# ccaven/tinyslam

Measured on AMD Instinct MI355X. Metric: ORB extract throughput, 1280x720 (frames/sec; Mkeypoints/sec alongside), higher is better.
Workload: dtype f32; 1 GPU; BASELINE.json configs[3]: batch of 256 independent 1280x720 RGBA frames per GPU, device-resident, full ORB (FAST-12 + orientation + blur + BRIEF-256); frames_per_gpu_per_batch=256, width=1280, height=720, hierarchy_depth=2, max_features=8192, content=default, mode=literal, input=rgba, pipeline=default, fp_contract=0, angle_bins=0, batches_in_flight=1, collate=none (1 GPU)

## Files before the change

tinyslam_amd/csrc/orb_api.hip:

```cpp
#include <hip/hip_runtime.h>
#include <chrono>
#include <cmath>

#include <cstdarg>
#include <cstdio>
#include <cstdlib>
#include <cstring>
#include <new>
#include <optional>
#include <string>
#include <algorithm>
#include <vector>

#include "../../include/tinyorb.h"
#include "orb_front_launch.h"
#include "orb_kernels_fused.h"
#include "orb_kernels_brief.h"
#include "orb_kernels_intended.h"
#include "orb_kernels_staged.h"
#include "orb_kernels_collate.h"
#include "orb_kernels_match.h"
#include "orb_kernels_verify.h"
#include "orb_kernels_epipolar.h"
#include "orb_kernels_guide.h"
// ... 84 lines not shown
    float* d_iseg_scores = nullptr;
    uint32_t* d_iseg_counts = nullptr;
    uint32_t* d_iseg_before = nullptr;
    unsigned long long* d_thr_key = nullptr;
    uint32_t ibrief_lds = 0;
    MatchRecord* d_matches = nullptr;
    uint8_t* d_desc8 = nullptr;
    int match_valu = -1;
    hipEvent_t match_done = nullptr;
    hipStream_t match_stream = nullptr;
    uint64_t batch_seq = 0;
    uint64_t match_seq = 0;
    uint32_t match_set = 0;
    uint32_t match_frames = 0;
    VerifierState verify, epi;
    uint4* d_gsrec = nullptr;
    uint4* d_gsdesc = nullptr;
    uint32_t* d_gcell = nullptr;
    MatchRecord* d_gmatch = nullptr;
    float* d_gmodel = nullptr;
    float* h_gmodel = nullptr;
    hipEvent_t guide_done = nullptr;
    hipStream_t guide_stream = nullptr;
    uint32_t guide_pairs = 0;
    int guide_cell = -1;
    uint64_t guide_seq = 0;
    uint32_t guide_set = 0;
    uint32_t* d_tkeys = nullptr;
    uint32_t* d_tprev = nullptr;
    uint32_t* d_tnext = nullptr;
    uint4* d_tptr = nullptr;
    uint4* d_track = nullptr;
    uint32_t* d_tlinks = nullptr;
    uint32_t* d_tshared = nullptr;
    uint32_t* d_tframe = nullptr;
    hipEvent_t track_done = nullptr;
    hipStream_t track_stream = nullptr;
    uint32_t track_frames = 0;
    int track_global_keys = -1;
    uint32_t* d_prov2_counts = nullptr;
    CornerData* d_prov2 = nullptr;
    float* d_prov2_scores = nullptr;

    uint8_t* d_input = nullptr;
    uint8_t* d_input_alt = nullptr;
    uint32_t in_last = 0;
    uint32_t in_pending = 0;
    uint32_t in_queue[2] = {0u, 0u};
    hipEvent_t in_uploaded[2] = {nullptr, nullptr};
    bool in_async[2] = {false, false};
    struct {
        bool single_memcpy = false, single_split = false, single_serial = false, single_sync = false, single_block = false;
        bool no_swizzle = false, quiet = false;
        int phase_mask = -1, brief_i_mask = -1, lds_pad = 0;
    } env;
    uint32_t* dv_count = nullptr;
    CornerData* dv_corners = nullptr;
    CornerDescriptor* dv_desc = nullptr;
    uint16_t* d_gray = nullptr;
    uint16_t* d_blur = nullptr;
    uint16_t* d_blur_rowc = nullptr;
    uint32_t blur_qa[kMaxLevels] = {0};
    uint32_t* d_counts = nullptr;
    CornerData* d_corners = nullptr;
    CornerDescriptor* d_desc = nullptr;
    uint32_t* out_counts[2] = {nullptr, nullptr};
    CornerData* out_corners[2] = {nullptr, nullptr};
    CornerDescriptor* out_desc[2] = {nullptr, nullptr};
    CornerData* d_seg = nullptr;
    uint32_t* d_seg_counts = nullptr;
    uint32_t* d_seg_before = nullptr;
    BandGeom bands{};
    RowsGeom rows{};
    BriefTGeom brieft{};
    bool use_brief_t = false;
    uint32_t band_rows_lvl[kMaxLevels] = {0};
    uint32_t ln_threads[kMaxLevels] = {0};
    uint32_t tile_w_lvl[kMaxLevels] = {0};
    uint32_t seg_classes = 1;
    uint32_t* d_pattern = nullptr;
    float* d_cos = nullptr;
    float* d_sin = nullptr;
    uint4* d_rot = nullptr;
    unsigned long long* d_stamps = nullptr;

    uint32_t* h_count = nullptr;
    uint32_t* d_single_done = nullptr;
    hipEvent_t single_done_ev = nullptr;
    uint32_t single_seq = 0;
    CornerData* h_corners = nullptr;
    CornerDescriptor* h_desc = nullptr;
    bool single_valid = false;

    uint32_t last_batch = 0;
    hipStream_t last_stream = nullptr;
    bool planes_valid = false;
    bool fused = false;
    uint32_t max_lds = 0;
    uint32_t n_cus = 256;

    bool profiling = false;
    std::vector<ProfSpan> pending;
    std::vector<hipEvent_t> event_pool;
    double prof_ms[ORB_KERNEL_COUNT] = {0};
    uint64_t prof_n[ORB_KERNEL_COUNT] = {0};

// ... 279 lines not shown
    g.rows_padded = rows;
    g.oob = p->oob;
    *out = g;
    if (getenv("TINYORB_BRIEF_ROWS")) return false;
    return rg.n_slots >= 1u && rg.n_slots * n_classes <= kBriefTMaxSlots && rows <= kBriefTMaxRows;
}

int launch_brief(OrbProgram* p, hipStream_t s, uint32_t n, const RowsGeom& rows_geom, const uint16_t* d_blur,
                 const uint16_t* d_blur_rowc, const uint32_t* seg_counts, uint32_t* seg_before, const CornerData* seg,
                 uint32_t* d_counts, CornerData* d_corners, CornerDescriptor* d_desc) {
    const uint32_t cap = p->cfg.max_features;
    const BriefTables tab{p->d_pattern, p->d_cos, p->d_sin, p->d_rot};
    const bool use_t = p->use_brief_t;
    {
        LaunchScope ls(p, s, KID_PREFIX);
        hipLaunchKernelGGL(k_slot_prefix, dim3(n), dim3(64), 0, s, seg_counts, seg_before, d_counts, rows_geom.n_slots,
                           rows_geom.seg_cap, use_t ? p->brieft.n_classes : 1u);
    }
    if (use_t) {
        const BriefTGeom& tg = p->brieft;
        const dim3 grid(n, (cap + (uint32_t)kBriefNfChunk - 1u) / (uint32_t)kBriefNfChunk);
        {
            LaunchScope ls(p, s, KID_BRIEF_T);
#define BRIEF_T_LAUNCH(ROT_)                                                                                                         \
    hipLaunchKernelGGL((k_brief_t<kBriefTWaves, ROT_>), dim3(n, (cap + kBriefTThreads - 1u) / kBriefTThreads), dim3(kBriefTThreads), \
                       brieft_lds_bytes(tg), s, d_blur_rowc, p->pyr, tg, seg_counts, seg_before, seg, d_corners, cap, d_desc, tab)
            switch (rot_form(p->opt.fp_contract)) {
                case 1: BRIEF_T_LAUNCH(1); break;
                case 2: BRIEF_T_LAUNCH(2); break;
                default: BRIEF_T_LAUNCH(0); break;
            }
#undef BRIEF_T_LAUNCH
        }
        LaunchScope ls(p, s, KID_BRIEF_NF);
        if (p->oob != kOobZero)
            hipLaunchKernelGGL(k_brief_nf<true>, grid, dim3(256), 0, s, d_blur, d_blur_rowc, p->pyr, tg, seg_counts, seg_before, d_corners,
                               cap, d_desc, tab);
        else
            hipLaunchKernelGGL(k_brief_nf<false>, grid, dim3(256), 0, s, d_blur, d_blur_rowc, p->pyr, tg, seg_counts, seg_before, d_corners,
                               cap, d_desc, tab);
    } else {
        LaunchScope ls(p, s, KID_BRIEF_ROWS);
        RowsGeom rg = rows_geom;
        rg.oob = p->oob;
        rg.fp = p->opt.fp_contract;
        rg.split = 1u;
        while (rg.split < 16u && rg.n_slots * n * rg.split < 2048u) rg.split *= 2u;
        hipLaunchKernelGGL(k_brief_rows, dim3(rg.n_slots * rg.split, n), dim3(256), 0, s, d_blur, d_blur_rowc, p->pyr, rg,
                           seg_counts, seg_before, seg, d_corners, cap, d_desc, tab);
    }
    return ORB_OK;
}

int run_fused_range(OrbProgram* p, const uint8_t* frames_all, uint32_t f0, uint32_t n, hipStream_t s, bool with_brief = true,
                    uint32_t first_level = 0) {
    const Pyramid& pyr = p->pyr;
    const uint32_t D = pyr.depth, cap = p->cfg.max_features;
    const uint8_t* frames = frames_all + (size_t)f0 * p->frame_bytes;
    uint16_t* const d_gray = p->d_gray + (size_t)f0 * pyr.stride;
    uint16_t* const d_blur = p->d_blur + (size_t)f0 * pyr.stride;
    uint16_t* const d_blur_rowc = p->d_blur_rowc + (size_t)f0 * pyr.row_stride;
    const size_t lists = (size_t)p->bands.n_slots * p->seg_classes;
    uint32_t* const d_seg_counts = p->d_seg_counts + (size_t)f0 * lists;
    uint32_t* const d_seg_before = p->d_seg_before + (size_t)f0 * lists;
    CornerData* const d_seg = p->d_seg + (size_t)f0 * lists * p->bands.seg_cap;
    uint32_t* const d_counts = p->d_counts + f0;
    CornerData* const d_corners = p->d_corners + (size_t)f0 * cap;
    CornerDescriptor* const d_desc = p->d_desc + (size_t)f0 * cap;
    uint32_t width = pyr.w[0], height = pyr.h[0];
    for (uint32_t lvl = 0; lvl < D; lvl++) {
        const uint32_t gw = ((width + 7u) / 8u) * 8u, gh = ((height + 7u) / 8u) * 8u;
        width /= 2u;
        height /= 2u;
        if (lvl < first_level) continue;
        if (lvl > 0 && !(pyr.w[lvl - 1] == 2u * pyr.w[lvl] && pyr.h[lvl - 1] == 2u * pyr.h[lvl])) {
            hipStream_t sm = s;
            LaunchScope ls(p, sm, KID_MIP);
            dim3 grid((pyr.w[lvl] + 63u) / 64u, (pyr.h[lvl] + 4u * kMipRows - 1u) / (4u * kMipRows), n);
            hipLaunchKernelGGL(k_mip, grid, dim3(64, 4), 0, sm, d_gray, pyr, lvl, (float)pyr.w[lvl - 1] / (float)pyr.w[lvl], (float)pyr.h[lvl - 1] / (float)pyr.h[lvl], p->wq);
        }
        FrontGeom g = front_geometry(pyr, lvl, gw ? gw : 8u, gh, n, p->band_rows_lvl[lvl], p->tile_w_lvl[lvl], p->ln_threads[lvl]);
        hipStream_t s_lvl = s;
        if (gw == 0) g.gh = 0;
        g.slot_base = p->bands.slot_base[lvl];
        g.n_slots = p->bands.n_slots;
        g.seg_cap = p->bands.seg_cap;
        g.n_classes = p->seg_classes;
        g.stamps = p->d_stamps;
        if (p->env.phase_mask >= 0) g.phase_mask = (uint32_t)p->env.phase_mask;
        if (p->env.no_swizzle) g.xcd_swizzle = 0u;
        g.oob = p->oob;
        g.wq = p->wq;
        g.fp = p->opt.fp_contract;
        g.store_grey = (lvl == 0 && D > 1 && !(pyr.w[0] == 2u * pyr.w[1] && pyr.h[0] == 2u * pyr.h[1])) ? 1u : 0u;
        if (g.n_bands * (g.tiled ? g.n_ct : 1u) != p->bands.slot_base[lvl + 1] - p->bands.slot_base[lvl])
            return fail(p, ORB_EINVAL, "internal: band count mismatch at level %u", lvl);
        if (!g.tiled && sizeof(BlurCol) * (size_t)g.n_var > 8u * (size_t)g.ts)
            return fail(p, ORB_EINVAL, "internal: blur column table of level %u does not fit", lvl);
        uint32_t lds = front_lds_bytes(g);
        lds += (uint32_t)p->env.lds_pad;
        if (lds > p->max_lds) return fail(p, ORB_EINVAL, "level %u needs %u bytes of LDS", lvl, lds);
        const dim3 grid(g.n_bands * (g.tiled ? g.n_ct : 1u) * n);
        FrontLaunch L{frames, p->frame_bytes, d_gray, d_blur, d_blur_rowc, pyr, g, p->threshold, d_seg_counts, d_seg, s_lvl, grid.x, lds,
                      p->band_rows_lvl[lvl], p->ln_threads[lvl], p->input_y8,
                      lvl == 0 && ((pyr.w[0] & 3u) || g.store_grey), p->oob != kOobZero, false};
        {
            LaunchScope ls(p, s_lvl, lvl == 0 ? KID_FUSED_L0 : KID_FUSED_LN);
            const hipError_t e = kFrontLaunch[front_form(p->opt.fp_contract, lvl == 0 && !p->input_y8)](L);
            if (e != hipSuccess) return fail(p, ORB_EHIP, "k_front (level %u) failed to launch: %s", lvl, hipGetErrorString(e));
        }
    }
    if (with_brief) launch_brief(p, s, n, p->rows, d_blur, d_blur_rowc, d_seg_counts, d_seg_before, d_seg, d_counts, d_corners, d_desc);
    HIP_TRY(p, hipGetLastError());
    return ORB_OK;
}

int run_fused(OrbProgram* p, const uint8_t* frames, uint32_t n, hipStream_t s) {
    if (int rc = run_fused_range(p, frames, 0, n, s)) return rc;
    p->planes_valid = true;
    return ORB_OK;
}

uint32_t itile_width(uint32_t w) {
    const uint32_t w8 = (w + 7u) & ~7u;
    return w8 < (uint32_t)kITileW ? w8 : (uint32_t)kITileW;
}

bool fused_i_eligible(const OrbProgram* p) {
    if (!p->intended || (p->opt.flags & ORB_FLAG_STAGED)) return false;
    const Pyramid& pyr = p->pyr;
    if ((uint64_t)pyr.w[0] * pyr.h[0] > (1ull << 26)) return false;
    if ((pyr.w[0] & 3u) != 0u || pyr.w[0] < 8u) return false;
    return true;
}

int run_fused_i(OrbProgram* p, const uint8_t* frames, uint32_t n, hipStream_t s) {
    const Pyramid& pyr = p->pyr;
    const uint32_t D = pyr.depth, cap = p->cfg.max_features;
    const IBriefGeom& bg = p->itiles;
    for (uint32_t lvl = 0; lvl < D; lvl++) {
        if (lvl > 0 && !(pyr.w[lvl - 1] == 2u * pyr.w[lvl] && pyr.h[lvl - 1] == 2u * pyr.h[lvl])) {
            LaunchScope ls(p, s, KID_MIP);
            dim3 grid((pyr.w[lvl] + 63u) / 64u, (pyr.h[lvl] + 4u * kMipRows - 1u) / (4u * kMipRows), n);
            hipLaunchKernelGGL(k_mip, grid, dim3(64, 4), 0, s, p->d_gray, pyr, lvl, (float)pyr.w[lvl - 1] / (float)pyr.w[lvl], (float)pyr.h[lvl - 1] / (float)pyr.h[lvl]);
        }
        IGeom g{};
        g.lvl = lvl;
        g.tw = bg.tw[lvl];
        g.n_ct = bg.n_ct[lvl];
        g.n_bands = (pyr.h[lvl] + kFrontRows - 1) / kFrontRows;
        g.ls = kIPad + g.tw + 16u;
        g.write_mip = (lvl + 1 < D && pyr.w[lvl] == 2u * pyr.w[lvl + 1] && pyr.h[lvl] == 2u * pyr.h[lvl + 1]) ? 1u : 0u;
        g.xcd_swizzle = (n % 8u == 0u) ? 1u : 0u;
        g.slot_base = bg.slot_base[lvl];
        g.n_slots = bg.n_slots;
        g.seg_cap = bg.seg_cap;
        g.arc = p->arc;
        g.nms = (p->opt.flags & ORB_FLAG_NMS) ? 1u : 0u;
// ... 175 lines not shown
    if (config->max_features == 0 || config->max_features > (1u << 24))
        return fail(nullptr, ORB_EINVAL, "max_features must be 1..=2^24");
    if (!(config->initial_threshold >= 0.f)) return fail(nullptr, ORB_EINVAL, "initial_threshold must be >= 0");
    if (options && options->fast_arc != 0 && (options->fast_arc < 9 || options->fast_arc > 16))
        return fail(nullptr, ORB_EINVAL, "fast_arc must be 0 (= 12) or 9..16");
    if (options && (options->flags & ORB_FLAG_INPUT_Y8) &&
        ((options->flags & (ORB_FLAG_INTENDED | ORB_FLAG_NMS)) || (options->fast_arc != 0 && options->fast_arc != 12)))
        return fail(nullptr, ORB_EINVAL, "ORB_FLAG_INPUT_Y8 is defined for the reference's detector only (no "
                                         "ORB_FLAG_INTENDED, ORB_FLAG_NMS or fast_arc other than 12)");
    if (options && (options->oob_policy > ORB_OOB_UMIN || options->sampler_weight_bits > 23u))
        return fail(nullptr, ORB_EINVAL, "oob_policy must be ORB_OOB_ZERO / _CLAMP / _UMIN and sampler_weight_bits 0..23");
    if (options && (options->oob_policy != ORB_OOB_ZERO || options->sampler_weight_bits != 0u) &&
        ((options->flags & (ORB_FLAG_INTENDED | ORB_FLAG_NMS)) || (options->fast_arc != 0 && options->fast_arc != 12)))
        return fail(nullptr, ORB_EINVAL, "oob_policy / sampler_weight_bits follow the reference's adapter: they are defined for the "
                                         "reference's detector only (no ORB_FLAG_INTENDED, ORB_FLAG_NMS or fast_arc other than 12)");
    if (options && options->fp_contract > (ORB_FP_CONTRACT_ALL | ORB_FP_LAST_TERM_FIRST))
        return fail(nullptr, ORB_EINVAL, "fp_contract is a mask of ORB_FP_CONTRACT_LUMINANCE / _BLUR / _ROTATION and ORB_FP_LAST_TERM_FIRST");
    if (options && options->fp_contract &&
        ((options->flags & (ORB_FLAG_INTENDED | ORB_FLAG_NMS | ORB_FLAG_INPUT_Y8)) || (options->fast_arc != 0 && options->fast_arc != 12)))
        return fail(nullptr, ORB_EINVAL, "fp_contract follows the reference's shader compiler: it is defined for the reference's detector on RGBA "
                                         "input only (no ORB_FLAG_INTENDED, ORB_FLAG_NMS, ORB_FLAG_INPUT_Y8 or fast_arc other than 12)");
    if (options && options->angle_bins && (!(options->flags & ORB_FLAG_INTENDED) || options->angle_bins < 8u || options->angle_bins > 6284u))
        return fail(nullptr, ORB_EINVAL, "angle_bins is an option of ORB_FLAG_INTENDED (IM-6b): 0, or 8..6284 bins of the full circle");
    if (options && (options->flags & ORB_FLAG_INTENDED) && (W > 16384u || H > 16384u))
        return fail(nullptr, ORB_EINVAL, "ORB_FLAG_INTENDED needs W, H <= 16384 (14-bit coordinates in the top-K key)");

    OrbProgram* p = new (std::nothrow) OrbProgram();
    if (!p) return fail(nullptr, ORB_EINVAL, "out of host memory");
    p->cfg = *config;
    if (options) p->opt = *options;
    p->device = p->opt.device;
    p->max_batch = p->opt.max_batch ? p->opt.max_batch : 1u;
    p->threshold = config->initial_threshold;
    p->intended = (p->opt.flags & ORB_FLAG_INTENDED) != 0u;
    p->input_y8 = (p->opt.flags & ORB_FLAG_INPUT_Y8) != 0u;
    p->arc = p->opt.fast_arc ? p->opt.fast_arc : (p->intended ? 9u : 12u);
    p->oob = p->opt.oob_policy;
    p->wq = p->opt.sampler_weight_bits ? (float)(1u << p->opt.sampler_weight_bits) : 0.0f;
    p->frame_bytes = (size_t)W * H * (p->input_y8 ? 1u : 4u);
    layout_pyramid(W, H, config->hierarchy_depth, &p->pyr);
    {
        auto on = [](const char* name) { const char* e = getenv(name); return e && *e && atoi(e) != 0; };
        auto num = [](const char* name, int dflt) { const char* e = getenv(name); return e && *e ? atoi(e) : dflt; };
        p->env.single_memcpy = on("TINYORB_SINGLE_MEMCPY");
        p->env.single_split = on("TINYORB_SINGLE_SPLIT");
        p->env.single_serial = on("TINYORB_SINGLE_SERIAL");
        p->env.single_sync = on("TINYORB_SINGLE_SYNC");
        {
            const char* w = getenv("TINYORB_SINGLE_WAIT");
            p->env.single_block = (w && !strcmp(w, "block")) || (p->opt.flags & ORB_FLAG_SINGLE_BLOCKING_WAIT) != 0u;
        }
        p->env.no_swizzle = on("TINYORB_NO_SWIZZLE");
        p->env.quiet = getenv("TINYORB_QUIET") != nullptr;
        p->env.phase_mask = num("TINYORB_PHASE_MASK", -1);
        p->env.brief_i_mask = num("TINYORB_BRIEF_I_MASK", -1);
        p->env.lds_pad = num("TINYORB_LDS_PAD", 0);
    }

    auto bail = [&](int code) {
        g_create_error = p->err;
        orb_program_destroy(p);
        return code;
    };
    int n_dev = 0;
    hipError_t e = hipGetDeviceCount(&n_dev);
    if (e != hipSuccess || n_dev <= 0) {
        fail(p, ORB_EHIP, "no HIP device available (%s)", e == hipSuccess ? "count is 0" : hipGetErrorString(e));
        return bail(ORB_EHIP);
    }
    if (p->device < 0 || p->device >= n_dev) {
        fail(p, ORB_EINVAL, "device %d out of range (0..%d)", p->device, n_dev - 1);
        return bail(ORB_EINVAL);
    }
#define CREATE_TRY(expr)                                                            \
    do {                                                                            \
        hipError_t e2_ = (expr);                                                    \
        if (e2_ != hipSuccess) {                                                    \
            fail(p, ORB_EHIP, "%s failed: %s", #expr, hipGetErrorString(e2_));      \
            return bail(ORB_EHIP);                                                  \
        }                                                                           \
    } while (0)
    CREATE_TRY(hipSetDevice(p->device));
    CREATE_TRY(hipStreamCreateWithFlags(&p->stream, hipStreamNonBlocking));
    {
        int lds_max = 0;
        CREATE_TRY(hipDeviceGetAttribute(&lds_max, hipDeviceAttributeMaxSharedMemoryPerBlock, p->device));
        p->max_lds = (uint32_t)lds_max;
        int cus = 0;
        CREATE_TRY(hipDeviceGetAttribute(&cus, hipDeviceAttributeMultiprocessorCount, p->device));
        p->n_cus = cus > 0 ? (uint32_t)cus : 256u;
        p->fused = fused_eligible(p);
        if (p->fused) {
            uint32_t need = 0;
            {
                uint32_t width = W, height = H;
                const char* force = getenv("TINYORB_BAND_ROWS");
                for (uint32_t lvl = 0; lvl < p->pyr.depth; lvl++) {
                    const uint32_t gw = ((width + 7u) / 8u) * 8u, gh = ((height + 7u) / 8u) * 8u, w = p->pyr.w[lvl];
                    width /= 2u;
                    height /= 2u;
                    uint32_t rows = 0, rows_lds = 0, fits = 0, fits_lds = 0, want = 0, want_lds = 0;
                    const uint32_t forced = force ? (uint32_t)atoi(force) : 0u;
                    auto pick = [&](uint32_t threads) {
                        rows = rows_lds = fits = fits_lds = want = want_lds = 0u;
                        for (int cand : kFrontBandHeights) {
                            if (std::max(w, gw) > (1u << front_x_bits(cand)) || std::max(w, gw) > (uint32_t)kFrontMaxWidthWide) continue;
// ... 28 lines not shown
                            tw = std::min(dom, (((dom + n_ct - 1u) / n_ct) + 7u) & ~7u);
                            t_rows = 0;
                            for (uint32_t cand : {16u, 8u}) {
                                const FrontGeom tg = front_geometry(p->pyr, lvl, gw, gh, 1, cand, tw);
                                const uint32_t lds = front_lds_bytes(tg);
                                const uint32_t items = lvl == 0 ? (tg.tw + 12u) / 4u : (tg.tw + 20u) / 8u;
                                if (!front_tile0_holds_blur(tg, w) || cand > (1u << (15u - tg.xb)) || lds > p->max_lds ||
                                    items > (lvl == 0 ? (uint32_t)kFrontThreadsL0 : (uint32_t)kFrontThreadsLN))
                                    continue;
                                if (!t_rows || (2u * lds <= p->max_lds && 2u * t_lds > p->max_lds)) t_rows = cand, t_lds = lds;
                                if (2u * t_lds <= p->max_lds) break;
                            }
                            if (t_rows || want_w >= dom) break;
                        }
                        if (t_rows) {
                            rows = t_rows, rows_lds = t_lds;
                            p->tile_w_lvl[lvl] = tw;
                        }
                    }
                    p->band_rows_lvl[lvl] = rows;
                    need = rows == 0 ? p->max_lds + 1u : std::max(need, rows_lds);
                }
            }
            if (need > p->max_lds) {
                p->fused = false;
            } else {
                BandGeom& bg = p->bands;
                uint32_t slots = 0;
                uint64_t band_px = 0;
                for (uint32_t lvl = 0; lvl < p->pyr.depth; lvl++) {
                    bg.slot_base[lvl] = slots;
                    const uint64_t lvl_cols = ((uint64_t)(W >> lvl) + 7u) / 8u * 8u;
                    uint32_t n_ct = 1;
                    if (p->tile_w_lvl[lvl]) n_ct = (uint32_t)((lvl_cols + p->tile_w_lvl[lvl] - 1u) / p->tile_w_lvl[lvl]);
                    slots += front_bands(p->pyr, lvl, p->band_rows_lvl[lvl]) * n_ct;
                    band_px = std::max<uint64_t>(band_px, (uint64_t)p->band_rows_lvl[lvl] * (p->tile_w_lvl[lvl] ? p->tile_w_lvl[lvl] : lvl_cols));
                }
                bg.slot_base[p->pyr.depth] = slots;
                bg.n_slots = slots;
                bg.seg_cap = (uint32_t)(band_px < config->max_features ? band_px : config->max_features);
                RowsGeom& rg = p->rows;
                rg.n_slots = bg.n_slots;
                rg.seg_cap = bg.seg_cap;
                for (uint32_t lvl = 0; lvl <= p->pyr.depth; lvl++) rg.slot_base[lvl] = bg.slot_base[lvl];
                for (uint32_t lvl = 0; lvl < p->pyr.depth; lvl++) {
                    const uint32_t q = front_geometry(p->pyr, lvl, 8, 8, 1).blur_q, qa = q & ~7u;
                    p->blur_qa[lvl] = qa;
                    rg.qa[lvl] = qa;
                    rg.flat_end[lvl] = q > (uint32_t)kBriefHalo ? q - kBriefHalo : 0u;
                }
                p->use_brief_t = brieft_geometry(p, rg, 2u, &p->brieft);
                p->seg_classes = p->use_brief_t ? 2u : 1u;
                for (auto set_max_lds : kFrontSetMaxLds) CREATE_TRY(set_max_lds((int)p->max_lds));
            }
        }
    }
    p->fused_i = fused_i_eligible(p);
    if (p->fused_i) {
        IBriefGeom& bg = p->itiles;
        uint32_t slots = 0;
        for (uint32_t lvl = 0; lvl < p->pyr.depth; lvl++) {
            bg.tw[lvl] = itile_width(p->pyr.w[lvl]);
            bg.n_ct[lvl] = (p->pyr.w[lvl] + bg.tw[lvl] - 1u) / bg.tw[lvl];
            bg.slot_base[lvl] = slots;
            slots += ((p->pyr.h[lvl] + kFrontRows - 1) / kFrontRows) * bg.n_ct[lvl];
        }
        bg.slot_base[p->pyr.depth] = slots;
        bg.n_slots = slots;
        uint32_t groups = 0, max_rows = 0;
        for (uint32_t lvl = 0; lvl < p->pyr.depth; lvl++) {
            bg.n_bands[lvl] = (p->pyr.h[lvl] + kFrontRows - 1) / kFrontRows;
            bg.group_base[lvl] = groups;
            groups += ((bg.n_bands[lvl] + kIBriefStack - 1) / kIBriefStack) * bg.n_ct[lvl];
            const uint32_t rows = std::min<uint32_t>(bg.n_bands[lvl], kIBriefStack) * kFrontRows + 2u * kBriefHalo;
            if (rows > max_rows) max_rows = rows;
        }
        bg.group_base[p->pyr.depth] = groups;
        p->igauss_fused = !getenv("TINYORB_I_GAUSS_KERNEL");
        for (uint32_t lvl = 0; lvl < p->pyr.depth; lvl++) p->igauss_fused = p->igauss_fused && ifront_gauss_fits(bg.tw[lvl]);
        p->igrey_stored = !p->igauss_fused || (p->pyr.depth > 1 && !(p->pyr.w[0] == 2u * p->pyr.w[1] && p->pyr.h[0] == 2u * p->pyr.h[1]));
        bg.seg_cap = (uint32_t)kFrontRows * bg.tw[0];
        bg.pitch = (uint32_t)kITileW + 2u * kIBriefApronX;
        p->ibrief_lds = max_rows * bg.pitch * (uint32_t)sizeof(uint16_t);
        hipFuncAttributes fa{};
        hipError_t ea = hipFuncGetAttributes(&fa, reinterpret_cast<const void*>(&k_brief_i));
        if (ea == hipSuccess && p->ibrief_lds + (uint32_t)fa.sharedSizeBytes > p->max_lds) {
            fail(p, ORB_EINVAL, "k_brief_i needs %u bytes of LDS", p->ibrief_lds + (uint32_t)fa.sharedSizeBytes);
            return bail(ORB_EINVAL);
        }
        if (ea == hipSuccess)
            ea = hipFuncSetAttribute(reinterpret_cast<const void*>(&k_brief_i), hipFuncAttributeMaxDynamicSharedMemorySize,
                                     (int)(p->max_lds - (uint32_t)fa.sharedSizeBytes));
        if (ea != hipSuccess) {
            fail(p, ORB_EHIP, "hipFuncSetAttribute(k_brief_i): %s", hipGetErrorString(ea));
            return bail(ORB_EHIP);
        }
    }
    p->fused_x = fused_x_eligible(p);
    if (p->fused_x) {
        IBriefGeom& bg = p->itiles;
        RowsGeom& rg = p->xrows;
        uint32_t slots = 0, bands = 0, need = 0;
        for (uint32_t lvl = 0; lvl < p->pyr.depth; lvl++) {
            uint32_t gw, gh;
            reference_grid(p->pyr, lvl, &gw, &gh);
            const uint32_t dw = std::max(p->pyr.w[lvl], gw), dh = std::max(p->pyr.h[lvl], gh);
// ... 1413 lines not shown
```

tinyslam_amd/csrc/orb_front_inst.hip:

```cpp
#include <hip/hip_runtime.h>

#include "orb_front_launch.h"

#ifndef TINYORB_FRONT_FP
#error "compile with -DTINYORB_FRONT_FP=0..7 (tinyslam_amd/build.py does)"
#endif

namespace orb {

namespace {
constexpr int FP = TINYORB_FRONT_FP;
constexpr int FPB = FP & 4;
constexpr bool kRest = (FP & 3) == 0;
}

#define ORB_CAT2(a, b) a##b
#define ORB_CAT(a, b) ORB_CAT2(a, b)
#define FRONT_ARGS L.frames, L.frame_bytes, L.gray, L.blur, L.blur_rowc, L.pyr, L.g, L.thr, L.seg_counts, L.segments
#define FRONT_GO(...) hipLaunchKernelGGL((k_front<__VA_ARGS__>), grid, block, L.lds, L.stream, FRONT_ARGS)
#define FRONT_BY_ROWS(PRE, POST)                                    \
    switch (L.band_rows) {                                          \
        case 64: FRONT_GO(PRE, 64, POST); break;                    \
        case 32: FRONT_GO(PRE, 32, POST); break;                    \
        case 16: FRONT_GO(PRE, 16, POST); break;                    \
        default: FRONT_GO(PRE, 8, POST); break;                     \
    }
#define FRONT_BY_ROWS_TILED(PRE, POST)                              \
    if (L.band_rows == 16u) FRONT_GO(PRE, 16, POST);                \
    else FRONT_GO(PRE, 8, POST);
#define COMMA ,

hipError_t ORB_CAT(front_launch_fp, TINYORB_FRONT_FP)(const FrontLaunch& L) {
    const dim3 grid(L.grid);
    const bool tiled = L.g.tiled != 0u;
    if (L.g.lvl == 0u && !L.input_y8 && !L.from_plane) {
        const dim3 block(kFrontThreadsL0);
        if (tiled && L.general) { FRONT_BY_ROWS_TILED(true COMMA false, true COMMA true COMMA false COMMA false COMMA 0 COMMA FP) }
        else if (tiled) { FRONT_BY_ROWS_TILED(true COMMA false, false COMMA true COMMA false COMMA false COMMA 0 COMMA FP) }
        else if (L.general) { FRONT_BY_ROWS(true COMMA false, true COMMA false COMMA false COMMA false COMMA 0 COMMA FP) }
        else { FRONT_BY_ROWS(true COMMA false, false COMMA false COMMA false COMMA false COMMA 0 COMMA FP) }
        return hipGetLastError();
    }
    if constexpr (kRest) {
        if (L.g.lvl == 0u && !L.from_plane) {
            const dim3 block(kFrontThreadsL0);
            if (tiled && L.general) { FRONT_BY_ROWS_TILED(true COMMA true, true COMMA true COMMA false COMMA false COMMA 0 COMMA FPB) }
            else if (tiled) { FRONT_BY_ROWS_TILED(true COMMA true, false COMMA true COMMA false COMMA false COMMA 0 COMMA FPB) }
            else if (L.general) { FRONT_BY_ROWS(true COMMA true, true COMMA false COMMA false COMMA false COMMA 0 COMMA FPB) }
            else { FRONT_BY_ROWS(true COMMA true, false COMMA false COMMA false COMMA false COMMA 0 COMMA FPB) }
        } else if (L.ln_threads == (uint32_t)kFrontThreadsLNBig) {
            const dim3 block(kFrontThreadsLNBig);
            FRONT_BY_ROWS(false COMMA false, false COMMA false COMMA false COMMA false COMMA kFrontThreadsLNBig COMMA FPB)
        } else {
            const dim3 block(kFrontThreadsLN);
            if (L.oob) {
                if (tiled) { FRONT_BY_ROWS_TILED(false COMMA false, false COMMA true COMMA false COMMA true COMMA 0 COMMA FPB) }
                else { FRONT_BY_ROWS(false COMMA false, false COMMA false COMMA false COMMA true COMMA 0 COMMA FPB) }
            } else if (tiled) { FRONT_BY_ROWS_TILED(false COMMA false, false COMMA true COMMA false COMMA false COMMA 0 COMMA FPB) }
            else { FRONT_BY_ROWS(false COMMA false, false COMMA false COMMA false COMMA false COMMA 0 COMMA FPB) }
        }
        return hipGetLastError();
    }
    return hipErrorInvalidValue;
}

hipError_t ORB_CAT(front_pair_launch_fp, TINYORB_FRONT_FP)(const FrontPairLaunch& L) {
    const dim3 grid(L.g0.n_bands + L.g1.n_bands), block(kFrontThreadsL0);
    if (!L.input_y8) {
        hipLaunchKernelGGL((k_front_pair<8, 8, false, FP>), grid, block, L.lds, L.stream, L.frames, L.frame_bytes, L.gray, L.blur, L.blur_rowc, L.pyr, L.g0,
                           L.g1, L.thr, L.seg_counts, L.segments);
        return hipGetLastError();
    }
    if constexpr (kRest) {
        hipLaunchKernelGGL((k_front_pair<8, 8, true, FPB>), grid, block, L.lds, L.stream, L.frames, L.frame_bytes, L.gray, L.blur, L.blur_rowc, L.pyr, L.g0,
                           L.g1, L.thr, L.seg_counts, L.segments);
        return hipGetLastError();
    }
    return hipErrorInvalidValue;
}

hipError_t ORB_CAT(front_set_max_lds_fp, TINYORB_FRONT_FP)(int max_lds) {
#define FN(...) reinterpret_cast<const void*>(&k_front<__VA_ARGS__>)
#define FN4(PRE, POST) FN(PRE, 64, POST), FN(PRE, 32, POST), FN(PRE, 16, POST), FN(PRE, 8, POST)
#define FN2(PRE, POST) FN(PRE, 16, POST), FN(PRE, 8, POST)
    const void* const rgba[] = {
        FN4(true COMMA false, false COMMA false COMMA false COMMA false COMMA 0 COMMA FP), FN4(true COMMA false, true COMMA false COMMA false COMMA false COMMA 0 COMMA FP),
        FN2(true COMMA false, false COMMA true COMMA false COMMA false COMMA 0 COMMA FP), FN2(true COMMA false, true COMMA true COMMA false COMMA false COMMA 0 COMMA FP),
        reinterpret_cast<const void*>(&k_front_pair<8, 8, false, FP>)};
    for (const void* f : rgba)
        if (hipError_t e = hipFuncSetAttribute(f, hipFuncAttributeMaxDynamicSharedMemorySize, max_lds)) return e;
    if constexpr (kRest) {
        const void* const rest[] = {
            FN4(true COMMA true, false COMMA false COMMA false COMMA false COMMA 0 COMMA FPB), FN4(true COMMA true, true COMMA false COMMA false COMMA false COMMA 0 COMMA FPB),
            FN2(true COMMA true, false COMMA true COMMA false COMMA false COMMA 0 COMMA FPB), FN2(true COMMA true, true COMMA true COMMA false COMMA false COMMA 0 COMMA FPB),
            FN4(false COMMA false, false COMMA false COMMA false COMMA false COMMA kFrontThreadsLNBig COMMA FPB),
            FN4(false COMMA false, false COMMA false COMMA false COMMA true COMMA 0 COMMA FPB), FN2(false COMMA false, false COMMA true COMMA false COMMA true COMMA 0 COMMA FPB),
            FN2(false COMMA false, false COMMA true COMMA false COMMA false COMMA 0 COMMA FPB), FN4(false COMMA false, false COMMA false COMMA false COMMA false COMMA 0 COMMA FPB),
            reinterpret_cast<const void*>(&k_front_pair<8, 8, true, FPB>)};
        for (const void* f : rest)
            if (hipError_t e = hipFuncSetAttribute(f, hipFuncAttributeMaxDynamicSharedMemorySize, max_lds)) return e;
    }
    return hipSuccess;
#undef FN
#undef FN4
#undef FN2
}

}
```

tinyslam_amd/csrc/orb_front_launch.h:

```cpp
#pragma once
#include "orb_kernels_front.h"

namespace orb {

struct FrontLaunch {
    const uint8_t* frames;
    size_t frame_bytes;
    uint16_t* gray;
    uint16_t* blur;
    uint16_t* blur_rowc;
    Pyramid pyr;
    FrontGeom g;
    float thr;
    uint32_t* seg_counts;
    CornerData* segments;
    hipStream_t stream;
    uint32_t grid;
    uint32_t lds;
    uint32_t band_rows;
    uint32_t ln_threads;
    bool input_y8;
    bool general;
    bool oob;
    bool from_plane;
};

struct FrontPairLaunch {
    const uint8_t* frames;
    size_t frame_bytes;
    uint16_t* gray;
    uint16_t* blur;
    uint16_t* blur_rowc;
    Pyramid pyr;
    FrontGeom g0, g1;
    float thr;
    uint32_t* seg_counts;
    CornerData* segments;
    hipStream_t stream;
    uint32_t lds;
    bool input_y8;
};

#define ORB_FRONT_DECL(F)                                        \
    hipError_t front_launch_fp##F(const FrontLaunch& L);         \
    hipError_t front_pair_launch_fp##F(const FrontPairLaunch& L); \
    hipError_t front_set_max_lds_fp##F(int max_lds);
ORB_FRONT_DECL(0) ORB_FRONT_DECL(1) ORB_FRONT_DECL(2) ORB_FRONT_DECL(3) ORB_FRONT_DECL(4) ORB_FRONT_DECL(5) ORB_FRONT_DECL(6) ORB_FRONT_DECL(7)
#undef ORB_FRONT_DECL

inline uint32_t front_form(uint32_t fp_contract, bool computes_luminance) {
    return (computes_luminance ? (uint32_t)lum_form(fp_contract) : 0u) | ((fp_contract & kFpBlur) ? 4u : 0u);
}

}
```

tinyslam_amd/csrc/orb_kernels_front.h:

```cpp
#pragma once
#include "../../include/tinyorb.h"
#include "orb_device.h"

namespace orb {

constexpr int kFrontThreadsL0 = 1024;
constexpr int kFrontThreadsLN = 512;
constexpr int kFrontThreadsLNBig = 1024;
constexpr int kFrontRows = 16;
constexpr int kFrontRowsWide = 8;
constexpr int kFrontTmpRows = 2;
constexpr int kFrontQueue = 4096;
constexpr int kFrontBandHeights[] = {64, 32, 16, 8};
__host__ __device__ constexpr int front_x_bits(int rows) { return rows == 64 ? 9 : rows == 32 ? 10 : rows == 16 ? 11 : 12; }
__host__ __device__ constexpr uint32_t front_mask_bit(int k, bool under) { return 1u << (8 * (k & 1) + (under ? 4 : 0) + (k >> 1)); }
constexpr int kFrontMaxWidth = 2048;
constexpr int kFrontMaxWidthWide = 4096;
constexpr int kFrontMaxWidthTiled = 16384;
constexpr int kFrontTileW = 1280;
constexpr int kLdsPad = 8;

struct FrontGeom {
    uint32_t lvl;
    uint32_t rows;
    uint32_t tiled;
    uint32_t tw;
    uint32_t n_ct;
    uint32_t xb;
    uint32_t far_i0, far_i1;
    uint32_t tmp_halfs;
    uint32_t gw, gh;
    uint32_t n_bands;
    uint32_t n_frames;
    uint32_t ls;
    uint32_t ts;
    uint32_t write_mip;
    uint32_t store_grey;
    uint32_t xcd_swizzle;
    uint32_t phase_mask;
    uint32_t slot_base;
    uint32_t n_slots;
    uint32_t seg_cap;
    uint32_t n_classes;
    uint32_t blur_p;
    uint32_t blur_q;
    uint32_t n_var;
    unsigned long long* stamps;
    uint32_t ovf_words;
    uint32_t oob;
    float wq;
    uint32_t fp;
};

struct __attribute__((aligned(8))) BlurCol {
    uint16_t a0, a1, b0, b1;
    float fa, fb, f2;
    uint32_t pad;
};
static_assert(sizeof(BlurCol) == 24, "BlurCol layout");

__host__ __device__ inline uint32_t front_lds_bytes(const FrontGeom& g) {
    if (g.tiled)
        return ((g.rows + 6) * g.ls + g.tmp_halfs) * 2u + kFrontQueue * 2u + 32u + 32u * g.rows + 8u * g.rows + 8u * g.ovf_words;
    return ((g.rows + 6) * g.ls + 2 * kFrontTmpRows * g.ts) * 2u + kFrontQueue * 2u + 32u + 32u * g.rows + 8u * g.ovf_words;
}

typedef float float4_t __attribute__((ext_vector_type(4)));
typedef float float3_t __attribute__((ext_vector_type(3)));
__device__ float4_t buffer_load_format_xyzw(__amdgpu_buffer_rsrc_t rsrc, int voffset, int soffset, int aux) __asm("llvm.amdgcn.raw.ptr.buffer.load.format.v4f32");
__device__ float3_t buffer_load_format_xyz(__amdgpu_buffer_rsrc_t rsrc, int voffset, int soffset, int aux) __asm("llvm.amdgcn.raw.ptr.buffer.load.format.v3f32");
constexpr int kBufferWord3Raw = 0x00020000;
constexpr int kBufferWord3Unorm8x4 = 0x00050FAC;

typedef unsigned short ushort2_t __attribute__((ext_vector_type(2)));
typedef float float2_t __attribute__((ext_vector_type(2)));
typedef _Float16 half2_t __attribute__((ext_vector_type(2)));
__device__ __forceinline__ ushort2_t as_u16x2(uint32_t v) { return __builtin_bit_cast(ushort2_t, v); }

__device__ __forceinline__ float h2f(uint32_t packed, int hi) {
    return from_half(bits_half((uint16_t)(hi ? (packed >> 16) : (packed & 0xffffu))));
}

__device__ __forceinline__ float unorm8_exact(float b) {
    const float rc_hi = 0x1.010102p-8f, rc_lo = -0x1.fdfdfep-33f;
    const float t = b * rc_lo;
    return __builtin_fmaf(b, rc_hi, t);
}
__device__ __forceinline__ float luminance_fast(uint32_t rgba) {
    float r = unorm8_exact((float)(rgba & 255u));
    float g = unorm8_exact((float)((rgba >> 8) & 255u));
    float b = unorm8_exact((float)((rgba >> 16) & 255u));
    float pr = 0.229f * r;
    float pg = 0.587f * g;
    float pb = 0.114f * b;
    return (pr + pg) + pb;
}
__device__ __forceinline__ uint32_t pack_half2(float lo, float hi) {
    return (uint32_t)half_bits(to_half(lo)) | ((uint32_t)half_bits(to_half(hi)) << 16);
}
template <bool BT601 = false, int LUM = 0>
__device__ __forceinline__ uint32_t luminance_pair_f16(uint32_t rgba0, uint32_t rgba1) {
    const float2_t rc_hi = {0x1.010102p-8f, 0x1.010102p-8f}, rc_lo = {-0x1.fdfdfep-33f, -0x1.fdfdfep-33f};
    const float2_t R = {(float)(rgba0 & 255u), (float)(rgba1 & 255u)};
    const float2_t G = {(float)((rgba0 >> 8) & 255u), (float)((rgba1 >> 8) & 255u)};
    const float2_t B = {(float)((rgba0 >> 16) & 255u), (float)((rgba1 >> 16) & 255u)};
    const float2_t tr = R * rc_lo, tb = B * rc_lo;
    const float2_t r = __builtin_elementwise_fma(R, rc_hi, tr);
    const float2_t b = __builtin_elementwise_fma(B, rc_hi, tb);
    constexpr float wr1 = BT601 ? 0.299f : 0.229f;
    const float2_t wr = {wr1, wr1}, wg = {0.587f, 0.587f}, wb = {0.114f, 0.114f};
    float2_t l;
    if constexpr (LUM == 1 || LUM == 3) {
// ... 101 lines not shown
        typedef short short2_t __attribute__((ext_vector_type(2)));
        const short2_t df = __builtin_bit_cast(short2_t, tt) - __builtin_bit_cast(short2_t, __builtin_bit_cast(uint32_t, v) ^ mm);
        const uint32_t sb = __builtin_bit_cast(uint32_t, __builtin_bit_cast(ushort2_t, df) >> (unsigned short)15);
        acc = j == 0 ? sb : ((sb << j) | acc);
    }
    const uint32_t mask = __builtin_amdgcn_perm(0u, acc, 0x0c0c0200u);
    return detect_streak_16(mask) != 0u;
}
__device__ __forceinline__ uint32_t ring_angle(const half_t* ctr, int ls) {
    float cx = 0.0f, cy = 0.0f;
#pragma unroll
    for (int i = 0; i < 16; i++) {
        const float v = from_half(ctr[kRingDy[i] * ls + kRingDx[i]]);
        const float px = v * (float)kRingDx[i];
        const float py = v * (float)kRingDy[i];
        cx = cx + px;
        cy = cy + py;
    }
    return angle_code(cy, cx);
}
__device__ __forceinline__ bool fast_full_test(const half_t* ctr, int ls, float thr, uint32_t* angle) {
    if (!ring_is_corner(ctr, ls, thr)) return false;
    *angle = ring_angle(ctr, ls);
    return true;
}
__device__ __forceinline__ bool diagonal_filter(const half_t* ctr, int ls, float thr, bool over) {
    const uint16_t a = half_bits(ctr[-2 * ls - 2]), b = half_bits(ctr[-2 * ls + 2]);
    const uint16_t d = half_bits(ctr[2 * ls - 2]), e = half_bits(ctr[2 * ls + 2]);
    const uint16_t lo1 = min(a, b), hi1 = max(a, b), lo2 = min(d, e), hi2 = max(d, e);
    const uint16_t m1 = max(lo1, lo2), m2 = min(hi1, hi2);
    const uint16_t sel = over ? min(m1, m2) : max(m1, m2);
    const float diff = from_half(bits_half(sel)) - from_half(ctr[0]);
    return over ? diff > thr : diff < -thr;
}

__device__ __forceinline__ void segment_append(bool is_corner, uint32_t x, uint32_t y, uint32_t angle, uint32_t oct,
                                               uint32_t* lds_counter, CornerData* seg, uint32_t seg_cap, bool two_lists) {
    if (is_corner) {
        const uint32_t cls = (two_lists && angle != 0u) ? 1u : 0u;
        const uint32_t idx = atomicAdd(lds_counter + cls, 1u);
        if (idx < seg_cap) *reinterpret_cast<uint4*>(&seg[cls * seg_cap + idx]) = make_uint4(x, y, angle, oct);
    }
}

template <bool L0, bool Y8 = false, int RB = kFrontRows, bool UA = false, bool TILED = false, bool SRC = false, int NTO = 0, bool OOBK = false, int FPF = 0>
__device__ __forceinline__ void front_body(const uint32_t block_id, const uint8_t* __restrict__ frames, size_t frame_bytes,
                                           uint16_t* __restrict__ gray, uint16_t* __restrict__ blur,
                                           uint16_t* __restrict__ blur_rowc, const Pyramid pyr,
                                           const FrontGeom geo, float thr, uint32_t* __restrict__ seg_counts,
                                           CornerData* __restrict__ segments) {
#include "orb_front_body.inc"
}

template <bool L0, bool Y8 = false, int RB = kFrontRows, bool UA = false, bool TILED = false, bool SRC = false, bool OOBK = false, int NTK = 0, int FPF = 0>
__global__ __launch_bounds__(NTK ? NTK : (L0 ? kFrontThreadsL0 : kFrontThreadsLN), (L0 || NTK == kFrontThreadsLNBig) ? 8 : 4) void k_front(const uint8_t* __restrict__ frames, size_t frame_bytes,
                                                         uint16_t* __restrict__ gray, uint16_t* __restrict__ blur,
                                                         uint16_t* __restrict__ blur_rowc, Pyramid pyr,
                                                         FrontGeom geo, float thr, uint32_t* __restrict__ seg_counts,
                                                         CornerData* __restrict__ segments) {
    constexpr int NTO = NTK;
    const uint32_t block_id = blockIdx.x;
#include "orb_front_body.inc"
}

template <int RB0, int RB1, bool Y8 = false, int FPF = 0>
__global__ __launch_bounds__(kFrontThreadsL0) void k_front_pair(const uint8_t* __restrict__ frames, size_t frame_bytes,
                                                              uint16_t* __restrict__ gray, uint16_t* __restrict__ blur,
                                                              uint16_t* __restrict__ blur_rowc, Pyramid pyr, FrontGeom geo0,
                                                              FrontGeom geo1, float thr, uint32_t* __restrict__ seg_counts,
                                                              CornerData* __restrict__ segments) {
    if (blockIdx.x < geo0.n_bands)
        front_body<true, Y8, RB0, false, false, false, 0, false, FPF>(blockIdx.x, frames, frame_bytes, gray, blur, blur_rowc, pyr, geo0, thr, seg_counts, segments);
    else
        front_body<false, Y8, RB1, false, false, true, kFrontThreadsL0, false, FPF>(blockIdx.x - geo0.n_bands, frames, frame_bytes, gray, blur, blur_rowc,
                                                                                   pyr, geo1, thr, seg_counts, segments);
}

}
```

Measured before the change: 497,400 frames/s.

## Specialise k_front instances with compile-time 720p geometry constants

```diff
diff --git a/tinyslam_amd/csrc/orb_api.hip b/tinyslam_amd/csrc/orb_api.hip
--- a/tinyslam_amd/csrc/orb_api.hip
+++ b/tinyslam_amd/csrc/orb_api.hip
@@ -160,6 +160,7 @@
     struct {
         bool single_memcpy = false, single_split = false, single_serial = false, single_sync = false, single_block = false;
         bool no_swizzle = false, quiet = false;
+        bool front_generic = false, front_trace = false;
         int phase_mask = -1, brief_i_mask = -1, lds_pad = 0;
     } env;
     uint32_t* dv_count = nullptr;
@@ -545,6 +546,43 @@
     return ORB_OK;
 }
 
+FrontGeom fused_level_geometry(const OrbProgram* p, uint32_t lvl, uint32_t gw, uint32_t gh, uint32_t n) {
+    const Pyramid& pyr = p->pyr;
+    FrontGeom g = front_geometry(pyr, lvl, gw ? gw : 8u, gh, n, p->band_rows_lvl[lvl], p->tile_w_lvl[lvl], p->ln_threads[lvl]);
+    if (gw == 0) g.gh = 0;
+    g.slot_base = p->bands.slot_base[lvl];
+    g.n_slots = p->bands.n_slots;
+    g.seg_cap = p->bands.seg_cap;
+    g.n_classes = p->seg_classes;
+    g.stamps = p->d_stamps;
+    if (p->env.phase_mask >= 0) g.phase_mask = (uint32_t)p->env.phase_mask;
+    if (p->env.no_swizzle) g.xcd_swizzle = 0u;
+    g.oob = p->oob;
+    g.wq = p->wq;
+    g.fp = p->opt.fp_contract;
+    g.store_grey = (lvl == 0 && pyr.depth > 1 && !(pyr.w[0] == 2u * pyr.w[1] && pyr.h[0] == 2u * pyr.h[1])) ? 1u : 0u;
+    return g;
+}
+
+FrontGeoId front_pick_geo(const OrbProgram* p, const FrontLaunch& L, const char** why = nullptr) {
+    const char* reason = nullptr;
+    FrontGeoId id = kFrontGeoGeneric;
+    const bool l0 = L.g.lvl == 0u;
+    if (p->env.front_generic) reason = "TINYORB_FRONT_GENERIC";
+    else if (L.g.lvl > 1u) reason = "lvl";
+    else if (L.input_y8) reason = "input_y8";
+    else if (L.general) reason = "general";
+    else if (L.oob) reason = "oob";
+    else if (L.from_plane) reason = "from_plane";
+    else if (front_form(p->opt.fp_contract, l0) != 0u) reason = "fp_contract";
+    else if (L.band_rows != (l0 ? FrontGeo720pL0::rows : FrontGeo720pL1::rows)) reason = "band_rows";
+    else if (!l0 && L.ln_threads != (uint32_t)kFrontThreadsLNBig) reason = "ln_threads";
+    else reason = l0 ? front_geo_mismatch<FrontGeo720pL0>(L.g, L.pyr) : front_geo_mismatch<FrontGeo720pL1>(L.g, L.pyr);
+    if (!reason) id = l0 ? kFrontGeo720pL0 : kFrontGeo720pL1;
+    if (why) *why = reason;
+    return id;
+}
+
 int run_fused_range(OrbProgram* p, const uint8_t* frames_all, uint32_t f0, uint32_t n, hipStream_t s, bool with_brief = true,
                     uint32_t first_level = 0) {
     const Pyramid& pyr = p->pyr;
@@ -572,20 +610,8 @@
             dim3 grid((pyr.w[lvl] + 63u) / 64u, (pyr.h[lvl] + 4u * kMipRows - 1u) / (4u * kMipRows), n);
             hipLaunchKernelGGL(k_mip, grid, dim3(64, 4), 0, sm, d_gray, pyr, lvl, (float)pyr.w[lvl - 1] / (float)pyr.w[lvl], (float)pyr.h[lvl - 1] / (float)pyr.h[lvl], p->wq);
         }
-        FrontGeom g = front_geometry(pyr, lvl, gw ? gw : 8u, gh, n, p->band_rows_lvl[lvl], p->tile_w_lvl[lvl], p->ln_threads[lvl]);
+        const FrontGeom g = fused_level_geometry(p, lvl, gw, gh, n);
         hipStream_t s_lvl = s;
-        if (gw == 0) g.gh = 0;
-        g.slot_base = p->bands.slot_base[lvl];
-        g.n_slots = p->bands.n_slots;
-        g.seg_cap = p->bands.seg_cap;
-        g.n_classes = p->seg_classes;
-        g.stamps = p->d_stamps;
-        if (p->env.phase_mask >= 0) g.phase_mask = (uint32_t)p->env.phase_mask;
-        if (p->env.no_swizzle) g.xcd_swizzle = 0u;
-        g.oob = p->oob;
-        g.wq = p->wq;
-        g.fp = p->opt.fp_contract;
-        g.store_grey = (lvl == 0 && D > 1 && !(pyr.w[0] == 2u * pyr.w[1] && pyr.h[0] == 2u * pyr.h[1])) ? 1u : 0u;
         if (g.n_bands * (g.tiled ? g.n_ct : 1u) != p->bands.slot_base[lvl + 1] - p->bands.slot_base[lvl])
             return fail(p, ORB_EINVAL, "internal: band count mismatch at level %u", lvl);
         if (!g.tiled && sizeof(BlurCol) * (size_t)g.n_var > 8u * (size_t)g.ts)
@@ -597,6 +623,7 @@
         FrontLaunch L{frames, p->frame_bytes, d_gray, d_blur, d_blur_rowc, pyr, g, p->threshold, d_seg_counts, d_seg, s_lvl, grid.x, lds,
                       p->band_rows_lvl[lvl], p->ln_threads[lvl], p->input_y8,
                       lvl == 0 && ((pyr.w[0] & 3u) || g.store_grey), p->oob != kOobZero, false};
+        L.geo = front_pick_geo(p, L);
         {
             LaunchScope ls(p, s_lvl, lvl == 0 ? KID_FUSED_L0 : KID_FUSED_LN);
             const hipError_t e = kFrontLaunch[front_form(p->opt.fp_contract, lvl == 0 && !p->input_y8)](L);
@@ -878,6 +905,8 @@
         }
         p->env.no_swizzle = on("TINYORB_NO_SWIZZLE");
         p->env.quiet = getenv("TINYORB_QUIET") != nullptr;
+        p->env.front_generic = on("TINYORB_FRONT_GENERIC");
+        p->env.front_trace = on("TINYORB_FRONT_TRACE");
         p->env.phase_mask = num("TINYORB_PHASE_MASK", -1);
         p->env.brief_i_mask = num("TINYORB_BRIEF_I_MASK", -1);
         p->env.lds_pad = num("TINYORB_LDS_PAD", 0);
@@ -1012,6 +1041,23 @@
                 p->use_brief_t = brieft_geometry(p, rg, 2u, &p->brieft);
                 p->seg_classes = p->use_brief_t ? 2u : 1u;
                 for (auto set_max_lds : kFrontSetMaxLds) CREATE_TRY(set_max_lds((int)p->max_lds));
+                if (p->env.front_trace) {
+                    uint32_t width = W, height = H;
+                    for (uint32_t lvl = 0; lvl < p->pyr.depth; lvl++) {
+                        const uint32_t gw = ((width + 7u) / 8u) * 8u, gh = ((height + 7u) / 8u) * 8u;
+                        width /= 2u;
+                        height /= 2u;
+                        const FrontGeom g = fused_level_geometry(p, lvl, gw, gh, p->max_batch);
+                        FrontLaunch L{};
+                        L.pyr = p->pyr, L.g = g, L.band_rows = p->band_rows_lvl[lvl], L.ln_threads = p->ln_threads[lvl], L.input_y8 = p->input_y8;
+                        L.general = lvl == 0 && ((p->pyr.w[0] & 3u) || g.store_grey), L.oob = p->oob != kOobZero;
+                        const char* why = nullptr;
+                        const FrontGeoId id = front_pick_geo(p, L, &why);
+                        fprintf(stderr, "tinyorb: k_front level %u (%ux%u, %u-row bands, batch %u) takes the %s instance%s%s\n", lvl, p->pyr.w[lvl], p->pyr.h[lvl],
+                                p->band_rows_lvl[lvl], p->max_batch, id == kFrontGeoGeneric ? "generic" : (id == kFrontGeo720pL0 ? "specialised 720p-L0" : "specialised 720p-L1"),
+                                why ? ": " : "", why ? why : "");
+                    }
+                }
             }
         }
     }
diff --git a/tinyslam_amd/csrc/orb_front_inst.hip b/tinyslam_amd/csrc/orb_front_inst.hip
--- a/tinyslam_amd/csrc/orb_front_inst.hip
+++ b/tinyslam_amd/csrc/orb_front_inst.hip
@@ -30,9 +30,29 @@
     else FRONT_GO(PRE, 8, POST);
 #define COMMA ,
 
+#if TINYORB_FRONT_FP == 0
+#define FRONT_GEO_L0 true, false, 16, false, false, false, false, 0, FP, FrontGeo720pL0
+#define FRONT_GEO_L1 false, false, 32, false, false, false, false, kFrontThreadsLNBig, FPB, FrontGeo720pL1
+#endif
+
 hipError_t ORB_CAT(front_launch_fp, TINYORB_FRONT_FP)(const FrontLaunch& L) {
     const dim3 grid(L.grid);
     const bool tiled = L.g.tiled != 0u;
+    if (L.geo != kFrontGeoGeneric) {
+#if TINYORB_FRONT_FP == 0
+        if (L.geo == kFrontGeo720pL0) {
+            const dim3 block(kFrontThreadsL0);
+            FRONT_GO(FRONT_GEO_L0);
+            return hipGetLastError();
+        }
+        if (L.geo == kFrontGeo720pL1) {
+            const dim3 block(kFrontThreadsLNBig);
+            FRONT_GO(FRONT_GEO_L1);
+            return hipGetLastError();
+        }
+#endif
+        return hipErrorInvalidValue;
+    }
     if (L.g.lvl == 0u && !L.input_y8 && !L.from_plane) {
         const dim3 block(kFrontThreadsL0);
         if (tiled && L.general) { FRONT_BY_ROWS_TILED(true COMMA false, true COMMA true COMMA false COMMA false COMMA 0 COMMA FP) }
@@ -89,6 +109,10 @@
         reinterpret_cast<const void*>(&k_front_pair<8, 8, false, FP>)};
     for (const void* f : rgba)
         if (hipError_t e = hipFuncSetAttribute(f, hipFuncAttributeMaxDynamicSharedMemorySize, max_lds)) return e;
+#if TINYORB_FRONT_FP == 0
+    for (const void* f : {FN(FRONT_GEO_L0), FN(FRONT_GEO_L1)})
+        if (hipError_t e = hipFuncSetAttribute(f, hipFuncAttributeMaxDynamicSharedMemorySize, max_lds)) return e;
+#endif
     if constexpr (kRest) {
         const void* const rest[] = {
             FN4(true COMMA true, false COMMA false COMMA false COMMA false COMMA 0 COMMA FPB), FN4(true COMMA true, true COMMA false COMMA false COMMA false COMMA 0 COMMA FPB),
diff --git a/tinyslam_amd/csrc/orb_front_launch.h b/tinyslam_amd/csrc/orb_front_launch.h
--- a/tinyslam_amd/csrc/orb_front_launch.h
+++ b/tinyslam_amd/csrc/orb_front_launch.h
@@ -2,6 +2,8 @@
 #include "orb_kernels_front.h"
 
 namespace orb {
+
+enum FrontGeoId : uint32_t { kFrontGeoGeneric = 0, kFrontGeo720pL0 = 1, kFrontGeo720pL1 = 2 };
 
 struct FrontLaunch {
     const uint8_t* frames;
@@ -23,6 +25,7 @@
     bool general;
     bool oob;
     bool from_plane;
+    FrontGeoId geo = kFrontGeoGeneric;
 };
 
 struct FrontPairLaunch {
diff --git a/tinyslam_amd/csrc/orb_kernels_front.h b/tinyslam_amd/csrc/orb_kernels_front.h
--- a/tinyslam_amd/csrc/orb_kernels_front.h
+++ b/tinyslam_amd/csrc/orb_kernels_front.h
@@ -58,6 +58,67 @@
     uint32_t pad;
 };
 static_assert(sizeof(BlurCol) == 24, "BlurCol layout");
+
+#define ORB_FRONT_GEO_FIELDS(X) \
+    X(lvl) X(rows) X(tiled) X(gw) X(gh) X(n_bands) X(ls) X(ts) X(write_mip) X(store_grey) X(xcd_swizzle) X(phase_mask) X(slot_base) \
+    X(n_slots) X(n_classes) X(blur_p) X(blur_q) X(n_var) X(ovf_words)
+struct FrontGeoNone {
+    static constexpr bool on = false;
+};
+struct FrontPyr720pD2 {
+    static constexpr uint32_t depth = 2, w0 = 1280, h0 = 720, w1 = 640, h1 = 360, off0 = 0, off1 = 1280 * 720, stride = 1280 * 720 + 640 * 360,
+                              row_off0 = 0, row_off1 = 720, row_stride = 1080;
+};
+struct FrontGeo720pL0 : FrontPyr720pD2 {
+    static constexpr bool on = true;
+    static constexpr uint32_t lvl = 0, rows = 16, tiled = 0, gw = 1280, gh = 720, n_bands = 45, ls = kLdsPad + 1288, ts = 1280, write_mip = 1,
+                              store_grey = 0, xcd_swizzle = 1, phase_mask = 15, slot_base = 0, n_slots = 45 + 12, n_classes = 2, blur_p = 563,
+                              blur_q = 1125, n_var = 1280 - 1125, ovf_words = 16 * 80 / 32;
+    static constexpr float wq = 0.0f;
+};
+struct FrontGeo720pL1 : FrontPyr720pD2 {
+    static constexpr bool on = true;
+    static constexpr uint32_t lvl = 1, rows = 32, tiled = 0, gw = 640, gh = 360, n_bands = 12, ls = kLdsPad + 648, ts = 640, write_mip = 0,
+                              store_grey = 0, xcd_swizzle = 1, phase_mask = 15, slot_base = 45, n_slots = 45 + 12, n_classes = 2, blur_p = 282,
+                              blur_q = 563, n_var = 640 - 563, ovf_words = 32 * 40 / 32;
+    static constexpr float wq = 0.0f;
+};
+template <class GEO>
+__host__ __device__ __forceinline__ FrontGeom front_geo_apply(FrontGeom g) {
+    if constexpr (GEO::on) {
+#define X(f) g.f = GEO::f;
+        ORB_FRONT_GEO_FIELDS(X)
+#undef X
+        g.wq = GEO::wq;
+    }
+    return g;
+}
+template <class GEO>
+__host__ __device__ __forceinline__ Pyramid front_pyr_apply(Pyramid p) {
+    if constexpr (GEO::on) {
+        p.depth = GEO::depth;
+        p.w[0] = GEO::w0, p.h[0] = GEO::h0, p.off[0] = GEO::off0, p.row_off[0] = GEO::row_off0;
+        p.w[1] = GEO::w1, p.h[1] = GEO::h1, p.off[1] = GEO::off1, p.row_off[1] = GEO::row_off1;
+        p.stride = GEO::stride, p.row_stride = GEO::row_stride;
+    }
+    return p;
+}
+template <class GEO>
+inline const char* front_geo_mismatch(const FrontGeom& g, const Pyramid& p) {
+#define X(f) \
+    if (g.f != GEO::f) return #f;
+    ORB_FRONT_GEO_FIELDS(X)
+#undef X
+    if (g.wq != GEO::wq) return "wq";
+    if (p.depth != GEO::depth) return "depth";
+    if (p.w[0] != GEO::w0 || p.w[1] != GEO::w1) return "w";
+    if (p.h[0] != GEO::h0 || p.h[1] != GEO::h1) return "h";
+    if (p.off[0] != GEO::off0 || p.off[1] != GEO::off1) return "off";
+    if (p.row_off[0] != GEO::row_off0 || p.row_off[1] != GEO::row_off1) return "row_off";
+    if (p.stride != GEO::stride) return "stride";
+    if (p.row_stride != GEO::row_stride) return "row_stride";
+    return nullptr;
+}
 
 __host__ __device__ inline uint32_t front_lds_bytes(const FrontGeom& g) {
     if (g.tiled)
@@ -265,14 +326,19 @@
 #include "orb_front_body.inc"
 }
 
-template <bool L0, bool Y8 = false, int RB = kFrontRows, bool UA = false, bool TILED = false, bool SRC = false, bool OOBK = false, int NTK = 0, int FPF = 0>
+template <bool L0, bool Y8 = false, int RB = kFrontRows, bool UA = false, bool TILED = false, bool SRC = false, bool OOBK = false, int NTK = 0, int FPF = 0,
+          class GEO = FrontGeoNone>
 __global__ __launch_bounds__(NTK ? NTK : (L0 ? kFrontThreadsL0 : kFrontThreadsLN), (L0 || NTK == kFrontThreadsLNBig) ? 8 : 4) void k_front(const uint8_t* __restrict__ frames, size_t frame_bytes,
                                                          uint16_t* __restrict__ gray, uint16_t* __restrict__ blur,
-                                                         uint16_t* __restrict__ blur_rowc, Pyramid pyr,
-                                                         FrontGeom geo, float thr, uint32_t* __restrict__ seg_counts,
+                                                         uint16_t* __restrict__ blur_rowc, Pyramid pyr_arg,
+                                                         FrontGeom geo_arg, float thr, uint32_t* __restrict__ seg_counts,
                                                          CornerData* __restrict__ segments) {
+    static_assert(!GEO::on || (!Y8 && !UA && !TILED && !SRC && !OOBK), "geometries exist for the aligned full-width kernels only");
+    if constexpr (GEO::on) static_assert((int)GEO::rows == RB && (GEO::lvl == 0u) == L0, "the geometry is of another instance");
     constexpr int NTO = NTK;
     const uint32_t block_id = blockIdx.x;
+    const Pyramid pyr = front_pyr_apply<GEO>(pyr_arg);
+    const FrontGeom geo = front_geo_apply<GEO>(geo_arg);
 #include "orb_front_body.inc"
 }
 
```

New measurement: 547,600 frames/s (median of 6 runs). 10.1% higher.
